# danielroe/ray-project-ray

Hardware: AMD Instinct MI355X
Metric: ray_train_gpt2_small_ddp_tokens_per_sec (higher is better)
Workload: dtype bf16

## Files before the change

### ray_amd/ops/_lib.py

```python

from __future__ import annotations

import ctypes
import os
import threading

_HERE = os.path.dirname(os.path.abspath(__file__))
LIB_PATH = os.path.join(os.path.dirname(_HERE), "_native", "libray_amd_hip.so")

_lib = None
_lock = threading.Lock()

c_void_p = ctypes.c_void_p
c_int = ctypes.c_int
c_long = ctypes.c_long
c_float = ctypes.c_float
c_double = ctypes.c_double
c_size_t = ctypes.c_size_t

_SIGS = {
    "ra_layernorm_fwd": [c_void_p] * 6 + [c_int, c_int, c_float, c_void_p],
    "ra_layernorm_bwd_parts": [c_int],
    "ra_layernorm_bwd": [c_void_p] * 11 + [c_int, c_int, c_int, c_void_p],
    "ra_residual_layernorm_fwd": [c_void_p] * 9 + [c_int, c_int, c_float, c_void_p],
# ... 34 lines not shown
    "ra_ppo_loss": [c_void_p] * 10 + [c_int, c_int] + [c_float] * 5 + [c_int, c_void_p],
    "ra_ppo_loss_packed": [c_void_p, c_void_p, c_void_p, c_int, c_int] + [c_void_p] * 4
                          + [c_int, c_int] + [c_float] * 5 + [c_void_p, c_int, c_float, c_void_p],
    "ra_scale_to_bf16": [c_void_p, c_long, c_void_p, c_void_p, c_void_p],
    "ra_ppo_heads_fwd": [c_void_p, c_int] + [c_void_p] * 5 + [c_int, c_int] + [c_void_p] * 3
                        + [c_int, c_int] + [c_float] * 5 + [c_void_p, c_float, c_void_p],
    "ra_ppo_heads_work": [c_int, c_int],
    "ra_ppo_heads_bwd": [c_void_p, c_int] + [c_void_p] * 10 + [c_int, c_int, c_int, c_void_p],
    "ra_c51_loss": [c_void_p] * 13 + [c_int, c_int, c_int, c_float, c_float, c_void_p],
    "ra_bias_relu_fwd": [c_void_p, c_void_p, c_void_p, c_long, c_int, c_void_p],
    "ra_relu_bwd_work": [c_int, c_int],
    "ra_relu_bwd_bias": [c_void_p] * 5 + [c_int, c_int, c_int, c_void_p],
    "ra_obsnorm_parts": [c_int],
    "ra_obsnorm_update": [c_void_p, c_int, c_int, c_double, c_void_p, c_void_p, c_void_p,
                          c_void_p],
    "ra_obsnorm_apply": [c_void_p] * 4 + [c_long, c_int, c_double, c_float, c_float, c_void_p],
    "ra_lt_num_cands": [c_int, c_int] + [c_long] * 6,
    "ra_lt_release_stream": [c_void_p],
    "ra_embed_bwd": [c_void_p] * 6 + [c_int, c_int, c_int, c_int, c_void_p],
    "ra_embed_bwd_work": [c_int, c_int, c_int],
    "ra_lt_num_streams": [],
    "ra_lt_set_choice": [c_int, c_int] + [c_long] * 6 + [c_int],
    "ra_lt_gemm": [c_int, c_int, c_long, c_long, c_long, c_void_p, c_long, c_void_p, c_long,
                   c_void_p, c_long, c_float, c_float, c_void_p],
    "ra_lt_tune": [c_int, c_int, c_long, c_long, c_long, c_void_p, c_long, c_void_p, c_long,
                   c_void_p, c_long, c_int, c_void_p, c_int, c_long, c_long, c_long, c_void_p],
    "ra_lt_gemm_batched": [c_int, c_int, c_long, c_long, c_long, c_void_p, c_long, c_long,
                           c_void_p, c_long, c_long, c_void_p, c_long, c_long, c_int, c_float,
                           c_float, c_void_p],
    "ra_lt_ep_num_cands": [c_int, c_int] + [c_long] * 6 + [c_int, c_long],
    "ra_lt_ep_set_choice": [c_int, c_int] + [c_long] * 6 + [c_int, c_long, c_int],
    "ra_lt_gemm_ep": [c_int, c_int, c_long, c_long, c_long, c_void_p, c_long, c_void_p, c_long,
                      c_void_p, c_long, c_int, c_void_p, c_void_p, c_long, c_int, c_void_p],
    "ra_lt_num_cands_batched": [c_int, c_int] + [c_long] * 6 + [c_int, c_long, c_long, c_long],
    "ra_lt_set_choice_batched": [c_int, c_int] + [c_long] * 6 + [c_int, c_long, c_long, c_long,
                                                                  c_int],
    "ra_lt_choice_name": [c_int, c_int] + [c_long] * 6 + [c_int, c_long, c_long, c_long,
                                                           ctypes.c_char_p, c_int],
    "ra_lt_allow_streamk": [c_int],
    "ra_lt_choice_is_streamk": [c_int, c_int] + [c_long] * 6 + [c_int, c_long, c_long, c_long],
    "ra_image_normalize": [c_void_p, c_void_p, c_int, c_int, c_int, c_int, c_void_p, c_void_p,
                           c_int, c_void_p],
    "ra_resize_bilinear": [c_void_p, c_void_p] + [c_int] * 6 + [c_void_p],
    "ra_cast_scale_u8": [c_void_p, c_void_p, c_long, c_float, c_void_p],
    "ra_gather_cast_u8": [c_void_p, c_void_p, c_void_p, c_long, c_long, c_float, c_void_p],
    "ra_conv_supported": [c_int] * 6,
    "ra_conv_fwd": [c_void_p, c_void_p, c_int, c_void_p, c_void_p, c_void_p] + [c_int] * 8
                   + [c_float, c_int, c_void_p],
    "ra_conv_wgrad_work": [c_int] * 8,
    "ra_conv_dgrad_supported": [c_int] * 5,
    "ra_conv_dgrad": [c_void_p] * 3 + [c_int] * 8 + [c_void_p],
    "ra_conv_wgrad": [c_void_p, c_void_p, c_int, c_void_p, c_void_p, c_long, c_void_p, c_int]
                     + [c_int] * 8 + [c_float, c_void_p],
    "ra_attn_fwd": [c_void_p, c_void_p, c_void_p, c_int, c_int, c_int, c_int, c_float,
                    c_void_p],
    "ra_attn_bwd": [c_void_p] * 6 + [c_int, c_int, c_int, c_int, c_float, c_void_p],
    "ra_attn_decode_splits": [c_int, c_int, c_int],
    "ra_attn_decode_work": [c_int, c_int, c_int, c_int],
    "ra_attn_decode": [c_void_p] * 6 + [c_int, c_int, c_int, c_float, c_int, c_void_p],
    "ra_kv_insert": [c_void_p] * 5 + [c_int] * 5 + [c_void_p],
    "ra_kv_copy": [c_void_p] * 7 + [c_int] * 7 + [c_void_p],
    "ra_attn_extend": [c_void_p] * 7 + [c_int] * 5 + [c_float, c_void_p],
    "ra_lora_add": [c_void_p] * 6 + [c_int] * 6 + [c_void_p],
    "ra_slot_advance": [c_void_p] * 6 + [c_int, c_int, c_long, c_void_p],
    "ra_sample_logits_max_v": [],
    "ra_sample_logits": [c_void_p, c_long] + [c_void_p] * 6 + [c_int, c_void_p, c_int, c_int,
# ... 66 lines not shown
```

### ray_amd/ops/csrc/gemm_lt.hip

```cpp
#include "common.h"

#include <hipblaslt/hipblaslt.h>
#include <hipblaslt/hipblaslt-ext.hpp>

#include <cstdlib>
#include <cstring>
#include <map>
#include <mutex>
#include <string>
#include <tuple>
#include <vector>

namespace {

typedef std::tuple<int, int, long, long, long, long, long, long, int, long, long, long> LtKey;

struct LtPlan {
  hipblasLtMatmulDesc_t desc = nullptr;
  hipblasLtMatrixLayout_t a = nullptr, b = nullptr, c = nullptr;
  std::vector<hipblasLtMatmulHeuristicResult_t> cands;
  std::vector<signed char> streamk;
  bool sk_only = false;
  int choice = 0;
};

hipblasLtHandle_t g_handle = nullptr;
const size_t kWs = 64ull << 20;
std::map<LtKey, LtPlan*> g_plans;
std::mutex g_mu;
std::map<hipStream_t, void*> g_ws_by_stream;
std::map<hipStream_t, hipblasLtHandle_t> g_handle_by_stream;
std::mutex g_ws_mu;

bool env_on(const char* name) {
  const char* e = getenv(name);
  return e && e[0] == '1';
}

hipblasLtHandle_t handle_for(hipStream_t st) {
  static const bool shared = env_on("RAY_AMD_LT_SHARED_HANDLE");
  if (shared) return g_handle;
  std::lock_guard<std::mutex> lk(g_ws_mu);
  auto it = g_handle_by_stream.find(st);
  if (it != g_handle_by_stream.end()) return it->second;
  hipblasLtHandle_t h = nullptr;
  if (hipblasLtCreate(&h) != HIPBLAS_STATUS_SUCCESS) return g_handle;
  g_handle_by_stream[st] = h;
  return h;
}

void* workspace(hipStream_t st) {
  std::lock_guard<std::mutex> lk(g_ws_mu);
// ... 180 lines not shown
RA_EXPORT void ra_lt_allow_streamk(int on) {
  std::lock_guard<std::mutex> g(g_mu);
  g_allow_sk = on != 0;
}

RA_EXPORT int ra_lt_release_stream(void* stream) {
  hipStream_t st = (hipStream_t)stream;
  std::lock_guard<std::mutex> lk(g_ws_mu);
  int freed = 0;
  auto w = g_ws_by_stream.find(st);
  auto h = g_handle_by_stream.find(st);
  if (w == g_ws_by_stream.end() && h == g_handle_by_stream.end()) return 0;
  hipStreamSynchronize(st);
  if (w != g_ws_by_stream.end()) {
    hipFree(w->second);
    g_ws_by_stream.erase(w);
    ++freed;
  }
  if (h != g_handle_by_stream.end()) {
    if (h->second != g_handle) hipblasLtDestroy(h->second);
    g_handle_by_stream.erase(h);
    ++freed;
  }
  return freed;
}

RA_EXPORT int ra_lt_num_streams() {
  std::lock_guard<std::mutex> lk(g_ws_mu);
  return (int)(g_ws_by_stream.size() > g_handle_by_stream.size() ? g_ws_by_stream.size()
                                                                   : g_handle_by_stream.size());
}

namespace {
typedef std::tuple<int, int, long, long, long, long, long, long, int, long> EpKey;
std::map<EpKey, LtPlan*> g_ep_plans;

LtPlan* get_ep_plan(int ta, int tb, long m, long n, long k, long lda, long ldb, long ldd, int ep,
                    long ldaux) {
  const EpKey key(ta, tb, m, n, k, lda, ldb, ldd, ep, ldaux);
  auto it = g_ep_plans.find(key);
  if (it != g_ep_plans.end()) return it->second;
  if (init_handle() != 0) return nullptr;
  LtPlan* p = new LtPlan();
  hipblasLtMatmulDescCreate(&p->desc, HIPBLAS_COMPUTE_32F, HIP_R_32F);
  hipblasOperation_t oa = ta ? HIPBLAS_OP_T : HIPBLAS_OP_N, ob = tb ? HIPBLAS_OP_T : HIPBLAS_OP_N;
  hipblasLtMatmulDescSetAttribute(p->desc, HIPBLASLT_MATMUL_DESC_TRANSA, &oa, sizeof(oa));
  hipblasLtMatmulDescSetAttribute(p->desc, HIPBLASLT_MATMUL_DESC_TRANSB, &ob, sizeof(ob));
  uint32_t e = (uint32_t)ep;
  hipblasLtMatmulDescSetAttribute(p->desc, HIPBLASLT_MATMUL_DESC_EPILOGUE, &e, sizeof(e));
  int32_t bt = ep == HIPBLASLT_EPILOGUE_DGELU_BGRAD ? HIP_R_32F : HIP_R_16BF;
  hipblasLtMatmulDescSetAttribute(p->desc, HIPBLASLT_MATMUL_DESC_BIAS_DATA_TYPE, &bt, sizeof(bt));
  int64_t la = ldaux;
  hipblasLtMatmulDescSetAttribute(p->desc, HIPBLASLT_MATMUL_DESC_EPILOGUE_AUX_LD, &la, sizeof(la));
  hipblasLtMatrixLayoutCreate(&p->a, HIP_R_16BF, ta ? k : m, ta ? m : k, lda);
  hipblasLtMatrixLayoutCreate(&p->b, HIP_R_16BF, tb ? n : k, tb ? k : n, ldb);
  hipblasLtMatrixLayoutCreate(&p->c, HIP_R_16BF, m, n, ldd);
  hipblasLtMatmulPreference_t pref;
  hipblasLtMatmulPreferenceCreate(&pref);
  uint64_t wsz = kWs;
  hipblasLtMatmulPreferenceSetAttribute(pref, HIPBLASLT_MATMUL_PREF_MAX_WORKSPACE_BYTES, &wsz,
                                        sizeof(wsz));
  std::vector<hipblasLtMatmulHeuristicResult_t> res(64);
  int got = 0;
  hipblasLtMatmulAlgoGetHeuristic(g_handle, p->desc, p->a, p->b, p->c, p->c, pref, 64,
                                  res.data(), &got);
  hipblasLtMatmulPreferenceDestroy(pref);
  for (int i = 0; i < got; ++i)
    if (res[i].state == HIPBLAS_STATUS_SUCCESS && res[i].workspaceSize <= kWs)
      p->cands.push_back(res[i]);
  g_ep_plans[key] = p;
  return p;
}
}

RA_EXPORT int ra_lt_ep_num_cands(int ta, int tb, long m, long n, long k, long lda, long ldb,
                                 long ldd, int ep, long ldaux) {
  std::lock_guard<std::mutex> g(g_mu);
  LtPlan* p = get_ep_plan(ta, tb, m, n, k, lda, ldb, ldd, ep, ldaux);
  return p ? (int)p->cands.size() : -1;
}

RA_EXPORT int ra_lt_ep_set_choice(int ta, int tb, long m, long n, long k, long lda, long ldb,
                                  long ldd, int ep, long ldaux, int choice) {
  std::lock_guard<std::mutex> g(g_mu);
  LtPlan* p = get_ep_plan(ta, tb, m, n, k, lda, ldb, ldd, ep, ldaux);
  if (!p || choice < 0 || choice >= (int)p->cands.size()) return -1;
  p->choice = choice;
  return 0;
}

RA_EXPORT int ra_lt_gemm_ep(int ta, int tb, long m, long n, long k, const void* A, long lda,
                            const void* B, long ldb, void* D, long ldd, int ep, void* bias,
                            void* aux, long ldaux, int choice, hipStream_t st) {
  LtPlan* p;
  {
    std::lock_guard<std::mutex> g(g_mu);
    p = get_ep_plan(ta, tb, m, n, k, lda, ldb, ldd, ep, ldaux);
    if (!p || p->cands.empty()) return -1;
    hipblasLtMatmulDescSetAttribute(p->desc, HIPBLASLT_MATMUL_DESC_BIAS_POINTER, &bias,
                                    sizeof(bias));
    hipblasLtMatmulDescSetAttribute(p->desc, HIPBLASLT_MATMUL_DESC_EPILOGUE_AUX_POINTER, &aux,
                                    sizeof(aux));
  }
  const int idx = choice >= 0 && choice < (int)p->cands.size() ? choice : p->choice;
  const float alpha = 1.f, beta = 0.f;
  const hipblasStatus_t s =
      hipblasLtMatmul(handle_for(st), p->desc, &alpha, A, p->a, B, p->b, &beta, D, p->c, D,
                      p->c, &p->cands[idx].algo, workspace(st), kWs, st);
  return s == HIPBLAS_STATUS_SUCCESS ? 0 : 1000 + (int)s;
}

RA_EXPORT int ra_lt_tune(int ta, int tb, long m, long n, long k, const void* A, long lda,
                         const void* B, long ldb, float* scratch, long ldc, int iters,
                         float* best_ms, int batch, long sa, long sb, long sc, hipStream_t st) {
  std::lock_guard<std::mutex> g(g_mu);
  LtPlan* p = get_plan(ta, tb, m, n, k, lda, ldb, ldc, batch, sa, sb, sc);
  if (!p || p->cands.empty()) return -1;
  hipEvent_t e0, e1;
  hipEventCreate(&e0);
  hipEventCreate(&e1);
  int best = -1;
  float bt = 1e30f;
  for (int i = 0; i < (int)p->cands.size(); ++i) {
    if (!usable(p, i)) continue;
    if (run(p, i, A, B, scratch, 1.f, 0.f, st) != 0) continue;
    hipEventRecord(e0, st);
    bool ok = true;
    for (int r = 0; r < iters && ok; ++r) ok = run(p, i, A, B, scratch, 1.f, 0.f, st) == 0;
    hipEventRecord(e1, st);
    hipEventSynchronize(e1);
    float ms = 0.f;
    hipEventElapsedTime(&ms, e0, e1);
    if (ok && ms / iters < bt) {
      bt = ms / iters;
      best = i;
    }
  }
  hipEventDestroy(e0);
  hipEventDestroy(e1);
  if (best >= 0) p->choice = best;
// ... 4 lines not shown
```

### ray_amd/ops/functional.py

```python

from __future__ import annotations

import os

import torch

from . import _lib
from . import reference as ref
from ._lib import check, ptr, stream_ptr


def _hip(t: torch.Tensor) -> bool:
    return t.is_cuda


def _grad_sink(p):
    if p is not None and getattr(p, "_ra_direct_grad", False):
        return getattr(p, "_ra_grad", None)
    return None


def _sink_f32(t) -> int:
    return 1 if t is not None and t.dtype == torch.float32 else 0

# ... 361 lines not shown
                getattr(w, "_ra_wt_key", None) == (_weights_epoch[0], w._version):
            return view, getattr(w, "_ra_wt_ev", None)
        side = _side_stream(w.device)
        side.wait_stream(torch.cuda.current_stream(w.device))
        with torch.cuda.stream(side):
            check(_lib.lib().ra_transpose_bf16(ptr(w), ptr(view), w.shape[0], w.shape[1],
                                               side.cuda_stream), "transpose_bf16")
            ev = torch.cuda.Event()
            ev.record(side)
        w._ra_wt_key = (_weights_epoch[0], w._version)
        w._ra_wt_ev = ev
        return view, ev
    cache = getattr(w, "_ra_wt", None)
    key = (_weights_epoch[0], w._version, w.data_ptr())
    stale = cache is None or cache[1] != key or torch.cuda.is_current_stream_capturing()
    if not stale:
        return cache[0], cache[2]
    wt = cache[0] if cache is not None else torch.empty(w.shape[1], w.shape[0], dtype=w.dtype,
                                                        device=w.device)
    side = _side_stream(w.device)
    side.wait_stream(torch.cuda.current_stream(w.device))
    with torch.cuda.stream(side):
        if w.dtype == torch.bfloat16 and w.dim() == 2 and w.is_contiguous():
            check(_lib.lib().ra_transpose_bf16(ptr(w), ptr(wt), w.shape[0], w.shape[1],
                                               side.cuda_stream), "transpose_bf16")
        else:
            wt.copy_(w.detach().t())
        ev = torch.cuda.Event()
        ev.record(side)
    w._ra_wt = (wt, key, ev)
    return wt, ev


class _Linear(torch.autograd.Function):
    @staticmethod
    def forward(ctx, x, w, b):
        ctx.save_for_backward(x, w)
        ctx.b = b
        ctx.wt = _transposed_weight(w) if _DGRAD_WT and w.is_cuda and x.dim() >= 2 else None
        return torch.nn.functional.linear(x, w, b)

    @staticmethod
    def backward(ctx, dy):
        x, w = ctx.saved_tensors
        K, N = x.shape[-1], w.shape[0]
        x2 = x.reshape(-1, K)
        dy2 = dy.reshape(-1, N)
        M = x2.shape[0]
        dx = None
        if ctx.needs_input_grad[0]:
            if ctx.wt is not None:
                wt, ev = ctx.wt
                if ev is not None:
                    torch.cuda.current_stream(dy2.device).wait_event(ev)
                dx = (dy2 @ wt.t()).view(x.shape)
            else:
                dx = (dy2 @ w).view(x.shape)
        dw = db = None
        bsink = None
        if ctx.b is not None and ctx.needs_input_grad[2] and ctx.needs_input_grad[1]:
            bsink = _grad_sink(ctx.b)
            ws_ = _grad_sink(w)
            if bsink is not None and (ws_ is None or ws_.dtype != bsink.dtype):
                bsink = None
        if ctx.needs_input_grad[1]:
            sink = _grad_sink(w)
            S = _splitk(M, N, K)
            if sink is not None and _WGRAD_STREAM and dy2.is_cuda:
                _issue_side_wgrad((dy2, x2, w, sink, S, M, N, K, ctx.b, bsink))
            elif sink is not None:
                _wgrad_to_sink(dy2, x2, w, sink, S, M, N, K, ctx.b, bsink)
            elif S > 1:
                part = _wgrad_partials(dy2, x2, S, M, N, K)
                dw = torch.empty_like(w)
                check(_lib.lib().ra_splitk_accum(ptr(part), S, N * K, ptr(dw), 2 * _sink_f32(dw),
                                                 stream_ptr()), "splitk_accum")
            else:
                dw = dy2.t() @ x2
        if ctx.b is not None and ctx.needs_input_grad[2] and bsink is None:
            db = _bias_grad(dy2, ctx.b)
        return dx, dw, db


def linear(x, w, b=None):
    if _hip(x) and x.dtype == torch.bfloat16 and w.dtype == torch.bfloat16 and \
            (w.shape[0] * w.shape[1]) % 4 == 0:
        return _Linear.apply(x, w, b)
    return torch.nn.functional.linear(x, w, b)


class _FlashAttnQKV(torch.autograd.Function):
    @staticmethod
    def forward(ctx, qkv, scale):
        B, T, _, H, D = qkv.shape
        qkv = qkv.contiguous()
        out = torch.empty((B, T, H, D), device=qkv.device, dtype=qkv.dtype)
        lse = torch.empty((B, H, T), device=qkv.device, dtype=torch.float32)
        check(_lib.lib().ra_attn_fwd(ptr(qkv), ptr(out), ptr(lse), B, T, H, D, scale,
                                     stream_ptr()), "attn_fwd")
        ctx.save_for_backward(qkv, out, lse)
        ctx.scale = scale
        return out

    @staticmethod
    def backward(ctx, dout):
        qkv, out, lse = ctx.saved_tensors
        B, T, _, H, D = qkv.shape
        dout = dout.contiguous()
        dqkv = torch.empty_like(qkv)
        delta = torch.empty((B, H, T), device=qkv.device, dtype=torch.float32)
        check(_lib.lib().ra_attn_bwd(ptr(qkv), ptr(out), ptr(dout), ptr(lse), ptr(delta),
                                     ptr(dqkv), B, T, H, D, ctx.scale, stream_ptr()),
              "attn_bwd")
        return dqkv, None
# ... 988 lines not shown
```

### ray_amd/ops/lt.py

```python

from __future__ import annotations

import ctypes
import os
import threading

import torch

from . import _lib
from ._lib import check, ptr, stream_ptr

_HERE = os.path.dirname(os.path.abspath(__file__))
DEFAULT_FILE = os.path.join(os.path.dirname(_HERE), "tuned", "lt_f32out.csv")

_lock = threading.Lock()
_choices: dict | None = None
_applied: set = set()
_tuning = os.environ.get("RAY_AMD_LT_TUNE", "0") == "1"
_file = os.environ.get("RAY_AMD_LT_FILE", DEFAULT_FILE)


def set_tuning(on: bool, path: str | None = None):
    global _tuning, _file
    _tuning = bool(on)
# ... 82 lines not shown

def gemm_f32(ta: int, tb: int, m: int, n: int, k: int, A, lda: int, B, ldb: int, C, ldc: int,
             alpha: float = 1.0, beta: float = 0.0, batch: int = 1, sa: int = 0, sb: int = 0,
             sc: int = 0):
    _select(ta, tb, m, n, k, ptr(A), lda, ptr(B), ldb, ldc, C.device, batch, sa, sb, sc)
    if batch == 1:
        rc = _lib.lib().ra_lt_gemm(ta, tb, m, n, k, ptr(A), lda, ptr(B), ldb, ptr(C), ldc,
                                   float(alpha), float(beta), stream_ptr())
    else:
        rc = _lib.lib().ra_lt_gemm_batched(ta, tb, m, n, k, ptr(A), lda, sa, ptr(B), ldb, sb,
                                           ptr(C), ldc, sc, batch, float(alpha), float(beta),
                                           stream_ptr())
    check(rc, "lt_gemm")


def wgrad_partials(dy2: torch.Tensor, x2: torch.Tensor, S: int) -> torch.Tensor:
    M, N = dy2.shape
    K = x2.shape[1]
    Ms = M // S
    part = torch.empty((S, N, K), dtype=torch.float32, device=dy2.device)
    gemm_f32(0, 1, K, N, Ms, x2, K, dy2, N, part, K, batch=S, sa=Ms * K, sb=Ms * N, sc=N * K)
    return part


def wgrad_accum(dy2: torch.Tensor, x2: torch.Tensor, out: torch.Tensor, beta: float = 1.0,
                alpha: float = 1.0):
    M, N = dy2.shape
    K = x2.shape[1]
    assert x2.shape[0] == M and out.shape == (N, K) and out.dtype == torch.float32
    assert dy2.stride(1) == 1 and x2.stride(1) == 1 and out.is_contiguous()
    gemm_f32(0, 1, K, N, M, x2, x2.stride(0), dy2, dy2.stride(0), out, K, alpha, beta)


def release_stream(stream) -> int:
    from ._lib import lib

    return int(lib().ra_lt_release_stream(stream.cuda_stream))
```

### ray_amd/ops/csrc/attn.hip

```cpp
#include "attn_mfma.h"

#include <type_traits>

#define HD 64
#define TILE_ELEMS (64 * 64)

__device__ __forceinline__ int xcd_block(int bid, int n) {
  return (n & 7) ? bid : (bid & 7) * (n >> 3) + (bid >> 3);
}

struct PairedBlock {
  int i, bh;
  bool two;
  __device__ __forceinline__ PairedBlock(int L, int nb) {
    const int np = (nb + 1) / 2;
    i = L % np;
    bh = L / np;
    two = nb - 1 - i != i;
  }
};

struct QD {
  TileRegs q, d;
  float rc;
};

__device__ __forceinline__ void tile_load(TileRegs& r, const bf16_t* g, long gstride) {
  const int c = threadIdx.x;
  r.v0 = *reinterpret_cast<const u32x4*>(g + (c >> 3) * gstride + (c & 7) * 8);
  r.v1 = *reinterpret_cast<const u32x4*>(g + ((c + 256) >> 3) * gstride + (c & 7) * 8);
}

struct TileAddr {
  int voff0, voff1;
  __device__ __forceinline__ TileAddr(long gstride) {
    const int c = threadIdx.x;
    voff0 = (int)(((c >> 3) * gstride + (c & 7) * 8) * 2);
    voff1 = (int)((((c + 256) >> 3) * gstride + (c & 7) * 8) * 2);
  }
};
__device__ __forceinline__ void tile_load_buf(TileRegs& r, __amdgpu_buffer_rsrc_t rs,
                                              const TileAddr& a, int soff) {
  r.v0 = __builtin_bit_cast(u32x4, __builtin_amdgcn_raw_buffer_load_b128(rs, a.voff0, soff, 0));
  r.v1 = __builtin_bit_cast(u32x4, __builtin_amdgcn_raw_buffer_load_b128(rs, a.voff1, soff, 0));
}


__device__ __forceinline__ int opaque_lane(int lane) {
  asm volatile("" : "+v"(lane));
  return lane;
}

__device__ __forceinline__ void store_rows_lds(bf16_t* img, const f32x16 (&acc)[2], float mul,
                                               bf16_t* g0, long gstride, int lane) {
  const int r = lane & 31, hh = lane >> 5;
#pragma unroll
  for (int dt = 0; dt < 2; ++dt)
// ... 88 lines not shown
  load_kv(A, 0);
  load_kv(B, 1);
  for (bool more = pb.two;; more = false) {
    store_kv(A, 0);
    kv_move(A, B);
    __syncthreads();
    for (int t = 0; t < ntiles; t += 2) {
      step(t, A, B);
      if (t + 1 < ntiles) step(t + 1, B, A);
    }
    if (more) {
      load_q(qf, pb.i, opaque_lane(lane));
      load_kv(A, 0);
      load_kv(B, 1);
    }
    static_assert(4 * 2048 <= 2 * TILE_ELEMS, "O staging must fit one tile buffer");
    const float inv = 1.f / l_run;
    store_rows_lds(lds + 2 * TILE_ELEMS + w * 2048, o, inv,
                   out + ((long)b * T + wave_qmin) * C + h * HD, C, opaque_lane(lane));
    if (hh == 0) lse[(long)bh * T + qrow] = m_run + log2f(l_run);
    if (!more) break;
    qb = pb.i;
    set_block();
  }
}

__global__ __launch_bounds__(256) __attribute__((amdgpu_waves_per_eu(2, 2))) void attn_bwd_dkdv_kernel(
    const bf16_t* __restrict__ qkv, const bf16_t* __restrict__ dout,
    const float* __restrict__ lse, const float* __restrict__ delta, bf16_t* __restrict__ dqkv,
    int T, int H, float sc_log2, float scale) {
  __shared__ __attribute__((aligned(16))) bf16_t lds[2 * 2 * TILE_ELEMS + 2 * 2 * 64 * 2];
  float* rowc = reinterpret_cast<float*>(lds + 4 * TILE_ELEMS);
  const int nkb = T / 128;
  const int L = xcd_block(blockIdx.x, gridDim.x);
  const int kb = L % nkb;
  const int bh = L / nkb;
  const int b = bh / H, h = bh % H;
  const int C = H * HD;
  const long tok = 3L * C;
  const bf16_t* base = qkv + (long)b * T * tok + h * HD;
  const bf16_t* dobase = dout + (long)b * T * C + h * HD;
  const int w = threadIdx.x >> 6, lane = threadIdx.x & 63, r = lane & 31, hh = lane >> 5;
  const LaneOffs lo(lane);
  const int kv0 = kb * 128;
  const int key = kv0 + 32 * w + r;
  bf16x8_t kf[4], vf[4];
#pragma unroll
  for (int kk = 0; kk < 4; ++kk) {
    kf[kk] = ld8(base + C + (long)key * tok + 16 * kk + 8 * hh);
    vf[kk] = ld8(base + 2 * C + (long)key * tok + 16 * kk + 8 * hh);
  }
  f32x16 dv[2] = {}, dk[2] = {};
  const int t0 = kv0 / 64;
  const int ntiles = T / 64;
  const int wave_kmin = kv0 + 32 * w;
  const float inv_c = -1.f / sc_log2;
  const float* lse_bh = lse + (long)bh * T;
  const float* del_bh = delta + (long)bh * T;
  QD A;
  const __amdgpu_buffer_rsrc_t rq = __builtin_amdgcn_make_buffer_rsrc(
      (void*)base, 0, (T - 1) * (int)tok * 2 + 3 * C * 2, 0x00020000);
  const __amdgpu_buffer_rsrc_t rd = __builtin_amdgcn_make_buffer_rsrc(
      (void*)dobase, 0, T * C * 2, 0x00020000);
  const TileAddr taq(tok), tad(C);
  const __amdgpu_buffer_rsrc_t rl =
      __builtin_amdgcn_make_buffer_rsrc((void*)lse_bh, 0, T * 4, 0x00020000);
  const __amdgpu_buffer_rsrc_t rdl =
      __builtin_amdgcn_make_buffer_rsrc((void*)del_bh, 0, T * 4, 0x00020000);
  auto load_qd = [&](QD& x, int t) __attribute__((always_inline)) {
    tile_load_buf(x.q, rq, taq, t * 64 * (int)tok * 2);
    tile_load_buf(x.d, rd, tad, t * 64 * C * 2);
    if (threadIdx.x < 128) {
      const float v = __builtin_bit_cast(
          float, __builtin_amdgcn_raw_buffer_load_b32(threadIdx.x < 64 ? rl : rdl,
                                                      (t * 64 + (threadIdx.x & 63)) * 4, 0, 0));
      x.rc = threadIdx.x < 64 ? v * inv_c : -v;
    }
  };
  auto store_qd = [&](const QD& x, int t) __attribute__((always_inline)) {
    const int buf = (t - t0) & 1;
    bf16_t* d = lds + buf * 2 * TILE_ELEMS;
    tile_store(x.q, d);
    tile_store(x.d, d + TILE_ELEMS);
    if (threadIdx.x < 128) rowc[buf * 128 + threadIdx.x] = x.rc;
  };
  auto body = [&](int t, auto diag_c) __attribute__((always_inline)) {
    constexpr bool diag = decltype(diag_c)::value;
    const int cur = (t - t0) & 1;
    const int q0 = t * 64;
    const bf16_t* Qs = lds + cur * 2 * TILE_ELEMS;
    const bf16_t* Ds = Qs + TILE_ELEMS;
    const float* nl = rowc + cur * 128;
    const float* nd = nl + 64;
    f32x16 s[2], dp[2];
#pragma unroll
    for (int qt = 0; qt < 2; ++qt) {
#pragma unroll
      for (int g = 0; g < 4; ++g) {
        const float4 a = *reinterpret_cast<const float4*>(nl + 32 * qt + 8 * g + 4 * hh);
        const float4 d = *reinterpret_cast<const float4*>(nd + 32 * qt + 8 * g + 4 * hh);
        s[qt][4 * g] = a.x; s[qt][4 * g + 1] = a.y; s[qt][4 * g + 2] = a.z;
        s[qt][4 * g + 3] = a.w;
        dp[qt][4 * g] = d.x; dp[qt][4 * g + 1] = d.y; dp[qt][4 * g + 2] = d.z;
        dp[qt][4 * g + 3] = d.w;
      }
#pragma unroll
      for (int kk = 0; kk < 4; ++kk) {
        s[qt] = mfma32(ld8(Qs + 2048 * qt + lo.row[kk]), kf[kk], s[qt]);
        dp[qt] = mfma32(ld8(Ds + 2048 * qt + lo.row[kk]), vf[kk], dp[qt]);
      }
    }
#pragma unroll
    for (int qt = 0; qt < 2; ++qt) {
#pragma unroll
      for (int i = 0; i < 16; ++i) {
        float p = fast_exp2(s[qt][i] * sc_log2);
        if (diag && key > q0 + 32 * qt + crow(i, hh)) p = 0.f;
        s[qt][i] = p;
        dp[qt][i] = p * dp[qt][i];
      }
#pragma unroll
      for (int ks = 0; ks < 2; ++ks) {
        const bf16x8_t pa = acc_frag(s[qt], ks);
        const bf16x8_t da = acc_frag(dp[qt], ks);
        const int kbq = 32 * qt + 16 * ks;
#pragma unroll
        for (int dt = 0; dt < 2; ++dt) {
          dv[dt] = mfma32(pa, tr_frag(Ds, lo, kbq, dt), dv[dt]);
          dk[dt] = mfma32(da, tr_frag(Qs, lo, kbq, dt), dk[dt]);
        }
      }
    }
  };
  auto compute = [&](int t) __attribute__((always_inline)) {
    const int q0 = t * 64;
    if (q0 + 63 >= wave_kmin) {
      if (q0 < wave_kmin + 31) body(t, std::true_type{});
      else body(t, std::false_type{});
    }
  };
  load_qd(A, t0);
  store_qd(A, t0);
  __syncthreads();
  for (int t = t0; t < ntiles; ++t) {
    if (t + 1 < ntiles) load_qd(A, t + 1);
    compute(t);
    if (t + 1 < ntiles) store_qd(A, t + 1);
    __syncthreads();
  }
#pragma unroll
  for (int dt = 0; dt < 2; ++dt)
#pragma unroll
    for (int i = 0; i < 16; ++i) {
      const int kr = kv0 + 32 * w + crow(i, hh);
      bf16_t* g = dqkv + ((long)b * T + kr) * tok + h * HD + 32 * dt + r;
      g[C] = f2bf(dk[dt][i] * scale);
      g[2 * C] = f2bf(dv[dt][i]);
    }
}

__global__ __launch_bounds__(256) void attn_bwd_dq_kernel(
    const bf16_t* __restrict__ qkv, const bf16_t* __restrict__ dout,
    const float* __restrict__ lse, float* __restrict__ delta, bf16_t* __restrict__ dqkv,
    int T, int H, float sc_log2, float scale, const bf16_t* __restrict__ out) {
  __shared__ __attribute__((aligned(16))) bf16_t lds[2 * 2 * TILE_ELEMS];
  const int nqb = T / 128;
  const PairedBlock pb(xcd_block(blockIdx.x, gridDim.x), nqb);
  const int bh = pb.bh;
  const int b = bh / H, h = bh % H;
  const int C = H * HD;
  const long tok = 3L * C;
  const bf16_t* base = qkv + (long)b * T * tok + h * HD;
  const int w = threadIdx.x >> 6, lane = threadIdx.x & 63, r = lane & 31, hh = lane >> 5;
  const LaneOffs lo(lane);
  struct RowIn {
    bf16x8_t q[4], d[4], o[4];
    float lse;
  };
  auto load_rows = [&](RowIn& x, int blk, int ln) __attribute__((always_inline)) {
    const int row = blk * 128 + 32 * w + (ln & 31), c0 = 8 * (ln >> 5);
#pragma unroll
    for (int kk = 0; kk < 4; ++kk) {
      x.q[kk] = ld8(base + (long)row * tok + 16 * kk + c0);
      x.d[kk] = ld8(dout + ((long)b * T + row) * C + h * HD + 16 * kk + c0);
      x.o[kk] = ld8(out + ((long)b * T + row) * C + h * HD + 16 * kk + c0);
    }
    x.lse = lse[(long)bh * T + row];
  };
  int q0, qrow, ntiles, wave_qmax;
  bf16x8_t qf[4], df[4];
  float nlq, ndel;
// ... 96 lines not shown
    RowIn x;
    if (more) {
      load_rows(x, pb.i, opaque_lane(lane));
      load_kv(A, 0);
      load_kv(B, 1);
    }
    store_rows_lds(lds + 2 * TILE_ELEMS + w * 2048, dq, scale,
                   dqkv + ((long)b * T + q0 + 32 * w) * tok + h * HD, tok, opaque_lane(lane));
    if (!more) break;
    set_block(pb.i, x);
  }
}

static inline bool attn_shape_ok(int T, int D) { return D == HD && T % 128 == 0 && T >= 128; }
static inline int attn_grid(int B, int T, int H) { return B * H * ((T / 128 + 1) / 2); }

RA_EXPORT int ra_attn_fwd(const void* qkv, void* out, float* lse, int B, int T, int H, int D,
                          float scale, hipStream_t st) {
  if (!attn_shape_ok(T, D)) return hipErrorInvalidValue;
  const float sc_log2 = scale * 1.4426950408889634f;
  hipLaunchKernelGGL(attn_fwd_kernel, dim3(attn_grid(B, T, H)), dim3(256), 0, st,
                     (const bf16_t*)qkv, (bf16_t*)out, lse, T, H, sc_log2);
  return hipGetLastError();
}

RA_EXPORT int ra_attn_bwd(const void* qkv, const void* out, const void* dout, const float* lse,
                          float* delta, void* dqkv, int B, int T, int H, int D, float scale,
                          hipStream_t st) {
  if (!attn_shape_ok(T, D)) return hipErrorInvalidValue;
  const float sc_log2 = scale * 1.4426950408889634f;
  hipLaunchKernelGGL(attn_bwd_dq_kernel, dim3(attn_grid(B, T, H)), dim3(256), 0, st,
                     (const bf16_t*)qkv, (const bf16_t*)dout, lse, delta, (bf16_t*)dqkv, T, H,
                     sc_log2, scale, (const bf16_t*)out);
  hipLaunchKernelGGL(attn_bwd_dkdv_kernel, dim3(B * H * (T / 128)), dim3(256), 0, st,
                     (const bf16_t*)qkv, (const bf16_t*)dout, lse, delta, (bf16_t*)dqkv, T, H,
                     sc_log2, scale);
  return hipGetLastError();
}
```

### ray_amd/ops/csrc/wgrad.hip

```cpp
#include "common.h"

namespace {

typedef __bf16 bf16x8w_t __attribute__((ext_vector_type(8)));
typedef __bf16 bf16x4w_t __attribute__((ext_vector_type(4)));
typedef __bf16 bf16x2w_t __attribute__((ext_vector_type(2)));
typedef short s16x4w_t __attribute__((ext_vector_type(4)));
typedef float f32x4w_t __attribute__((ext_vector_type(4)));
typedef __attribute__((address_space(3))) void lds_void_w;
typedef __attribute__((address_space(1))) void glb_void_w;

constexpr int kT = 64;
constexpr int kTile = 256;
constexpr int kImg = kT * kTile;
constexpr int kStage = 2 * kImg;
constexpr int kThreads = 512;

__device__ __forceinline__ int fsw(int r) { return (r & 3) | ((r >> 1) & 4); }

__device__ __forceinline__ bf16x4w_t tr4(const bf16_t* p) {
  typedef __attribute__((address_space(3))) s16x4w_t lds_s16x4;
  s16x4w_t v = __builtin_amdgcn_ds_read_tr16_b64_v4i16((lds_s16x4*)const_cast<bf16_t*>(p));
  return __builtin_bit_cast(bf16x4w_t, v);
}

__device__ __forceinline__ int xcd_remap_w(int b, int G) {
  const int q = G / 8, rr = G % 8, x = b % 8;
  return (x < rr ? x * (q + 1) : rr * (q + 1) + (x - rr) * q) + b / 8;
}

__device__ __forceinline__ void glds16_w(const bf16_t* gsrc, bf16_t* ldst) {
  const unsigned la = __builtin_amdgcn_readfirstlane(
      (unsigned)(unsigned long)(__attribute__((address_space(3))) void*)ldst);
  unsigned saved;
  asm volatile(
      "s_mov_b32 %0, m0\n\t"
      "s_mov_b32 m0, %2\n\t"
      "s_nop 0\n\t"
      "global_load_lds_dwordx4 %1, off\n\t"
      "s_mov_b32 m0, %0"
      : "=&s"(saved)
      : "v"(gsrc), "s"(la)
      : "memory");
}

template <int N>
__device__ __forceinline__ void wait_vm_w() {
  asm volatile("s_waitcnt vmcnt(%0)" ::"n"(N) : "memory");
}

struct WgradArgs {
  const bf16_t* dy;
  const bf16_t* x;
  long ldy, ldx;
  void* out;
  float* bias_out;
  int N, K, nks;
  int S, tk_cnt, ntiles;
  int flags;
};

__device__ __forceinline__ void stage_t(bf16_t* img, const bf16_t* __restrict__ g, long ld,
                                        int col0, int cols, long t0, int w, int lane) {
  const int rsub = lane >> 5, cp = lane & 31;
#pragma unroll
  for (int j = 0; j < 4; ++j) {
    const int r = 8 * w + 2 * j + rsub;
    const int c = cp ^ (2 * fsw(r));
    int col = col0 + 8 * c;
    col = col < cols ? col : cols - 8;
    const bf16_t* src = g + (t0 + r) * ld + col;
    glds16_w(src, img + (8 * w + 2 * j) * kTile);
  }
}

struct TileJob {
  const bf16_t* dy;
  const bf16_t* x;
  long ldy, ldx;
  int N, K, n0, k0, s_beg, total;
  bool do_bias;
};
// ... 276 lines not shown
```

Measured before the change: 1.066 million.

## Add hipBLASLt GEMM with bias and residual-add epilogue for linear layers

Adds a hipBLASLt matmul path that computes out = W·y + bias + skip in one call, using beta=1 with a separate C input layout and a bias epilogue. The autograd function and the linear_residual helper let projection layers fold the residual add into the GEMM. The aim is to remove a separate bias-plus-residual elementwise kernel and its memory traffic. The backward pass reuses the shared linear backward and passes dy through to the skip input. It adds candidate tuning and plan caching keyed on ldc.

Result: slower. 879,500 (-17.5%).

```diff
diff --git a/ray_amd/ops/_lib.py b/ray_amd/ops/_lib.py
--- a/ray_amd/ops/_lib.py
+++ b/ray_amd/ops/_lib.py
@@ -90,6 +90,10 @@
     "ra_lt_ep_set_choice": [c_int, c_int] + [c_long] * 6 + [c_int, c_long, c_int],
     "ra_lt_gemm_ep": [c_int, c_int, c_long, c_long, c_long, c_void_p, c_long, c_void_p, c_long,
                       c_void_p, c_long, c_int, c_void_p, c_void_p, c_long, c_int, c_void_p],
+    "ra_lt_res_num_cands": [c_int, c_int] + [c_long] * 7,
+    "ra_lt_res_set_choice": [c_int, c_int] + [c_long] * 7 + [c_int],
+    "ra_lt_gemm_res": [c_int, c_int, c_long, c_long, c_long, c_void_p, c_long, c_void_p, c_long,
+                       c_void_p, c_long, c_void_p, c_long, c_void_p, c_int, c_void_p],
     "ra_lt_num_cands_batched": [c_int, c_int] + [c_long] * 6 + [c_int, c_long, c_long, c_long],
     "ra_lt_set_choice_batched": [c_int, c_int] + [c_long] * 6 + [c_int, c_long, c_long, c_long,
                                                                   c_int],
diff --git a/ray_amd/ops/csrc/gemm_lt.hip b/ray_amd/ops/csrc/gemm_lt.hip
--- a/ray_amd/ops/csrc/gemm_lt.hip
+++ b/ray_amd/ops/csrc/gemm_lt.hip
@@ -18,6 +18,7 @@
 struct LtPlan {
   hipblasLtMatmulDesc_t desc = nullptr;
   hipblasLtMatrixLayout_t a = nullptr, b = nullptr, c = nullptr;
+  hipblasLtMatrixLayout_t cin = nullptr;
   std::vector<hipblasLtMatmulHeuristicResult_t> cands;
   std::vector<signed char> streamk;
   bool sk_only = false;
@@ -264,12 +265,12 @@
 }
 
 namespace {
-typedef std::tuple<int, int, long, long, long, long, long, long, int, long> EpKey;
+typedef std::tuple<int, int, long, long, long, long, long, long, int, long, long> EpKey;
 std::map<EpKey, LtPlan*> g_ep_plans;
 
 LtPlan* get_ep_plan(int ta, int tb, long m, long n, long k, long lda, long ldb, long ldd, int ep,
-                    long ldaux) {
-  const EpKey key(ta, tb, m, n, k, lda, ldb, ldd, ep, ldaux);
+                    long ldaux, long ldc = 0) {
+  const EpKey key(ta, tb, m, n, k, lda, ldb, ldd, ep, ldaux, ldc);
   auto it = g_ep_plans.find(key);
   if (it != g_ep_plans.end()) return it->second;
   if (init_handle() != 0) return nullptr;
@@ -283,10 +284,13 @@
   int32_t bt = ep == HIPBLASLT_EPILOGUE_DGELU_BGRAD ? HIP_R_32F : HIP_R_16BF;
   hipblasLtMatmulDescSetAttribute(p->desc, HIPBLASLT_MATMUL_DESC_BIAS_DATA_TYPE, &bt, sizeof(bt));
   int64_t la = ldaux;
-  hipblasLtMatmulDescSetAttribute(p->desc, HIPBLASLT_MATMUL_DESC_EPILOGUE_AUX_LD, &la, sizeof(la));
+  if (ldaux > 0)
+    hipblasLtMatmulDescSetAttribute(p->desc, HIPBLASLT_MATMUL_DESC_EPILOGUE_AUX_LD, &la,
+                                    sizeof(la));
   hipblasLtMatrixLayoutCreate(&p->a, HIP_R_16BF, ta ? k : m, ta ? m : k, lda);
   hipblasLtMatrixLayoutCreate(&p->b, HIP_R_16BF, tb ? n : k, tb ? k : n, ldb);
   hipblasLtMatrixLayoutCreate(&p->c, HIP_R_16BF, m, n, ldd);
+  if (ldc > 0) hipblasLtMatrixLayoutCreate(&p->cin, HIP_R_16BF, m, n, ldc);
   hipblasLtMatmulPreference_t pref;
   hipblasLtMatmulPreferenceCreate(&pref);
   uint64_t wsz = kWs;
@@ -294,8 +298,8 @@
                                         sizeof(wsz));
   std::vector<hipblasLtMatmulHeuristicResult_t> res(64);
   int got = 0;
-  hipblasLtMatmulAlgoGetHeuristic(g_handle, p->desc, p->a, p->b, p->c, p->c, pref, 64,
-                                  res.data(), &got);
+  hipblasLtMatmulAlgoGetHeuristic(g_handle, p->desc, p->a, p->b, p->cin ? p->cin : p->c, p->c,
+                                  pref, 64, res.data(), &got);
   hipblasLtMatmulPreferenceDestroy(pref);
   for (int i = 0; i < got; ++i)
     if (res[i].state == HIPBLAS_STATUS_SUCCESS && res[i].workspaceSize <= kWs)
@@ -338,6 +342,41 @@
   const float alpha = 1.f, beta = 0.f;
   const hipblasStatus_t s =
       hipblasLtMatmul(handle_for(st), p->desc, &alpha, A, p->a, B, p->b, &beta, D, p->c, D,
+                      p->c, &p->cands[idx].algo, workspace(st), kWs, st);
+  return s == HIPBLAS_STATUS_SUCCESS ? 0 : 1000 + (int)s;
+}
+
+static const int kResEp = HIPBLASLT_EPILOGUE_BIAS;
+
+RA_EXPORT int ra_lt_res_num_cands(int ta, int tb, long m, long n, long k, long lda, long ldb,
+                                  long ldc, long ldd) {
+  std::lock_guard<std::mutex> g(g_mu);
+  LtPlan* p = ldc > 0 ? get_ep_plan(ta, tb, m, n, k, lda, ldb, ldd, kResEp, 0, ldc) : nullptr;
+  return p ? (int)p->cands.size() : -1;
+}
+
+RA_EXPORT int ra_lt_res_set_choice(int ta, int tb, long m, long n, long k, long lda, long ldb,
+                                   long ldc, long ldd, int choice) {
+  std::lock_guard<std::mutex> g(g_mu);
+  LtPlan* p = ldc > 0 ? get_ep_plan(ta, tb, m, n, k, lda, ldb, ldd, kResEp, 0, ldc) : nullptr;
+  if (!p || choice < 0 || choice >= (int)p->cands.size()) return -1;
+  p->choice = choice;
+  return 0;
+}
+
+RA_EXPORT int ra_lt_gemm_res(int ta, int tb, long m, long n, long k, const void* A, long lda,
+                             const void* B, long ldb, const void* C, long ldc, void* D, long ldd,
+                             const void* bias, int choice, hipStream_t st) {
+  if (ldc <= 0 || !A || !B || !C || !D || !bias || D == C) return -1;
+  std::lock_guard<std::mutex> g(g_mu);
+  LtPlan* p = get_ep_plan(ta, tb, m, n, k, lda, ldb, ldd, kResEp, 0, ldc);
+  if (!p || p->cands.empty()) return -1;
+  hipblasLtMatmulDescSetAttribute(p->desc, HIPBLASLT_MATMUL_DESC_BIAS_POINTER, &bias,
+                                  sizeof(bias));
+  const int idx = choice >= 0 && choice < (int)p->cands.size() ? choice : p->choice;
+  const float alpha = 1.f, beta = 1.f;
+  const hipblasStatus_t s =
+      hipblasLtMatmul(handle_for(st), p->desc, &alpha, A, p->a, B, p->b, &beta, C, p->cin, D,
                       p->c, &p->cands[idx].algo, workspace(st), kWs, st);
   return s == HIPBLAS_STATUS_SUCCESS ? 0 : 1000 + (int)s;
 }
diff --git a/ray_amd/ops/functional.py b/ray_amd/ops/functional.py
--- a/ray_amd/ops/functional.py
+++ b/ray_amd/ops/functional.py
@@ -417,6 +417,47 @@
     return wt, ev
 
 
+def _linear_backward(ctx, dy):
+    x, w = ctx.saved_tensors
+    K, N = x.shape[-1], w.shape[0]
+    x2 = x.reshape(-1, K)
+    dy2 = dy.reshape(-1, N)
+    M = x2.shape[0]
+    dx = None
+    if ctx.needs_input_grad[0]:
+        if ctx.wt is not None:
+            wt, ev = ctx.wt
+            if ev is not None:
+                torch.cuda.current_stream(dy2.device).wait_event(ev)
+            dx = (dy2 @ wt.t()).view(x.shape)
+        else:
+            dx = (dy2 @ w).view(x.shape)
+    dw = db = None
+    bsink = None
+    if ctx.b is not None and ctx.needs_input_grad[2] and ctx.needs_input_grad[1]:
+        bsink = _grad_sink(ctx.b)
+        ws_ = _grad_sink(w)
+        if bsink is not None and (ws_ is None or ws_.dtype != bsink.dtype):
+            bsink = None
+    if ctx.needs_input_grad[1]:
+        sink = _grad_sink(w)
+        S = _splitk(M, N, K)
+        if sink is not None and _WGRAD_STREAM and dy2.is_cuda:
+            _issue_side_wgrad((dy2, x2, w, sink, S, M, N, K, ctx.b, bsink))
+        elif sink is not None:
+            _wgrad_to_sink(dy2, x2, w, sink, S, M, N, K, ctx.b, bsink)
+        elif S > 1:
+            part = _wgrad_partials(dy2, x2, S, M, N, K)
+            dw = torch.empty_like(w)
+            check(_lib.lib().ra_splitk_accum(ptr(part), S, N * K, ptr(dw), 2 * _sink_f32(dw),
+                                             stream_ptr()), "splitk_accum")
+        else:
+            dw = dy2.t() @ x2
+    if ctx.b is not None and ctx.needs_input_grad[2] and bsink is None:
+        db = _bias_grad(dy2, ctx.b)
+    return dx, dw, db
+
+
 class _Linear(torch.autograd.Function):
     @staticmethod
     def forward(ctx, x, w, b):
@@ -427,44 +468,45 @@
 
     @staticmethod
     def backward(ctx, dy):
-        x, w = ctx.saved_tensors
-        K, N = x.shape[-1], w.shape[0]
-        x2 = x.reshape(-1, K)
-        dy2 = dy.reshape(-1, N)
-        M = x2.shape[0]
-        dx = None
-        if ctx.needs_input_grad[0]:
-            if ctx.wt is not None:
-                wt, ev = ctx.wt
-                if ev is not None:
-                    torch.cuda.current_stream(dy2.device).wait_event(ev)
-                dx = (dy2 @ wt.t()).view(x.shape)
-            else:
-                dx = (dy2 @ w).view(x.shape)
-        dw = db = None
-        bsink = None
-        if ctx.b is not None and ctx.needs_input_grad[2] and ctx.needs_input_grad[1]:
-            bsink = _grad_sink(ctx.b)
-            ws_ = _grad_sink(w)
-            if bsink is not None and (ws_ is None or ws_.dtype != bsink.dtype):
-                bsink = None
-        if ctx.needs_input_grad[1]:
-            sink = _grad_sink(w)
-            S = _splitk(M, N, K)
-            if sink is not None and _WGRAD_STREAM and dy2.is_cuda:
-                _issue_side_wgrad((dy2, x2, w, sink, S, M, N, K, ctx.b, bsink))
-            elif sink is not None:
-                _wgrad_to_sink(dy2, x2, w, sink, S, M, N, K, ctx.b, bsink)
-            elif S > 1:
-                part = _wgrad_partials(dy2, x2, S, M, N, K)
-                dw = torch.empty_like(w)
-                check(_lib.lib().ra_splitk_accum(ptr(part), S, N * K, ptr(dw), 2 * _sink_f32(dw),
-                                                 stream_ptr()), "splitk_accum")
-            else:
-                dw = dy2.t() @ x2
-        if ctx.b is not None and ctx.needs_input_grad[2] and bsink is None:
-            db = _bias_grad(dy2, ctx.b)
-        return dx, dw, db
+        return _linear_backward(ctx, dy)
+
+
+class _LinearResidual(torch.autograd.Function):
+
+    @staticmethod
+    def forward(ctx, y, w, b, skip):
+        from . import lt
+
+        ctx.save_for_backward(y, w)
+        ctx.b = b
+        ctx.wt = _transposed_weight(w) if _DGRAD_WT else None
+        out = lt.gemm_bias_residual(y.reshape(-1, y.shape[-1]), w, b,
+                                    skip.reshape(-1, w.shape[0]))
+        return out.view(skip.shape)
+
+    @staticmethod
+    def backward(ctx, dy):
+        return _linear_backward(ctx, dy) + (dy,)
+
+
+def linear_residual_ok(y, w, b, skip) -> bool:
+    if not (_hip(y) and b is not None and w.dim() == 2 and y.dim() >= 2
+            and y.dtype == w.dtype == b.dtype == skip.dtype == torch.bfloat16
+            and skip.is_cuda and y.shape[-1] == w.shape[1] and skip.shape[-1] == w.shape[0]
+            and skip.shape[:-1] == y.shape[:-1]
+            and y.is_contiguous() and w.is_contiguous() and skip.is_contiguous()
+            and b.is_contiguous() and w.shape[0] % 8 == 0 and w.shape[1] % 8 == 0):
+        return False
+    from . import lt
+
+    return lt.residual_ready(y.numel() // y.shape[-1], w.shape[0], w.shape[1])
+
+
+def linear_residual(y, w, b, skip):
+    if linear_residual_ok(y, w, b, skip):
+        return _LinearResidual.apply(y, w, b, skip)
+    h = linear(y, w)
+    return bias_residual(h, b, skip) if b is not None else h + skip
 
 
 def linear(x, w, b=None):
diff --git a/ray_amd/ops/lt.py b/ray_amd/ops/lt.py
--- a/ray_amd/ops/lt.py
+++ b/ray_amd/ops/lt.py
@@ -138,6 +138,75 @@
     gemm_f32(0, 1, K, N, M, x2, x2.stride(0), dy2, dy2.stride(0), out, K, alpha, beta)
 
 
+def _res_shape(M: int, N: int, K: int):
+    return (1, 0, N, M, K, K, K, N, N)
+
+
+def _res_key(shape) -> str:
+    return "lt_res_" + "_".join(map(str, shape[2:]))
+
+
+def residual_num_cands(M: int, N: int, K: int) -> int:
+    return int(_lib.lib().ra_lt_res_num_cands(*_res_shape(M, N, K)))
+
+
+def residual_ready(M: int, N: int, K: int) -> bool:
+    if residual_num_cands(M, N, K) <= 0:
+        return False
+    return _res_key(_res_shape(M, N, K)) in _applied or \
+        not torch.cuda.is_current_stream_capturing()
+
+
+def _select_res(shape, key, a2, w, bias, skip2, out):
+    if key in _applied:
+        return
+    with _lock:
+        if key in _applied:
+            return
+        L = _lib.lib()
+        nc = L.ra_lt_res_num_cands(*shape)
+        if nc <= 0:
+            raise RuntimeError(f"hipBLASLt has no solution for {key}")
+        ch = _load()
+        if key in ch and ch[key][0] < nc and L.ra_lt_res_set_choice(*shape, ch[key][0]) == 0:
+            pass
+        elif _tuning:
+            ta, tb, m, n, k, lda, ldb, ldc, ldd = shape
+            args = (ta, tb, m, n, k, ptr(w), lda, ptr(a2), ldb, ptr(skip2), ldc, ptr(out), ldd,
+                    ptr(bias))
+            best, best_ms = -1, float("inf")
+            e0, e1 = torch.cuda.Event(enable_timing=True), torch.cuda.Event(enable_timing=True)
+            for i in range(nc):
+                if L.ra_lt_gemm_res(*args, i, stream_ptr()) != 0:
+                    continue
+                e0.record()
+                ok = all(L.ra_lt_gemm_res(*args, i, stream_ptr()) == 0 for _ in range(5))
+                e1.record()
+                e1.synchronize()
+                if ok and e0.elapsed_time(e1) / 5 < best_ms:
+                    best, best_ms = i, e0.elapsed_time(e1) / 5
+            if best >= 0 and L.ra_lt_res_set_choice(*shape, best) == 0:
+                ch[key] = (best, best_ms)
+        _applied.add(key)
+
+
+def gemm_bias_residual(a2: torch.Tensor, w: torch.Tensor, bias: torch.Tensor,
+                       skip2: torch.Tensor) -> torch.Tensor:
+    M, K = a2.shape
+    N = w.shape[0]
+    assert w.shape == (N, K) and bias.shape == (N,) and skip2.shape == (M, N)
+    assert a2.is_contiguous() and w.is_contiguous() and skip2.is_contiguous() and \
+        bias.is_contiguous()
+    assert a2.dtype == w.dtype == bias.dtype == skip2.dtype == torch.bfloat16
+    out = torch.empty_like(skip2)
+    shape = _res_shape(M, N, K)
+    _select_res(shape, _res_key(shape), a2, w, bias, skip2, out)
+    ta, tb, m, n, k, lda, ldb, ldc, ldd = shape
+    check(_lib.lib().ra_lt_gemm_res(ta, tb, m, n, k, ptr(w), lda, ptr(a2), ldb, ptr(skip2), ldc,
+                                    ptr(out), ldd, ptr(bias), -1, stream_ptr()), "lt_gemm_res")
+    return out
+
+
 def release_stream(stream) -> int:
     from ._lib import lib
 
```

## Pair causal key blocks and stream Q/dO tiles via LDS DMA in dK/dV kernel

Applied to the files above, without the earlier changes.

Reworks the attention backward dK/dV kernel so each workgroup handles a pair of key blocks (i and nkb-1-i), which balances the causal triangle's uneven work and halves the grid. Q and dO tiles now go from global memory straight into LDS through global_load_lds DMA instead of passing through registers, and the next block's K/V fragments and first tile are prefetched while the current block's results are written out. The shared DMA helpers move into a common header. The risks are correctness of the swizzled DMA addressing and of the partial vmcnt wait, plus lower parallelism from the smaller grid.

After: 1.070 million tokens/s before, 1.077 million tokens/s after, median of 6. Within noise of the previous version (+0.7%).

```diff
diff --git a/ray_amd/ops/csrc/attn.hip b/ray_amd/ops/csrc/attn.hip
--- a/ray_amd/ops/csrc/attn.hip
+++ b/ray_amd/ops/csrc/attn.hip
@@ -1,4 +1,5 @@
 #include "attn_mfma.h"
+#include "lds_dma.h"
 
 #include <type_traits>
 
@@ -18,11 +19,6 @@
     bh = L / np;
     two = nb - 1 - i != i;
   }
-};
-
-struct QD {
-  TileRegs q, d;
-  float rc;
 };
 
 __device__ __forceinline__ void tile_load(TileRegs& r, const bf16_t* g, long gstride) {
@@ -177,57 +173,61 @@
   __shared__ __attribute__((aligned(16))) bf16_t lds[2 * 2 * TILE_ELEMS + 2 * 2 * 64 * 2];
   float* rowc = reinterpret_cast<float*>(lds + 4 * TILE_ELEMS);
   const int nkb = T / 128;
-  const int L = xcd_block(blockIdx.x, gridDim.x);
-  const int kb = L % nkb;
-  const int bh = L / nkb;
+  const PairedBlock pb(xcd_block(blockIdx.x, gridDim.x), nkb);
+  const int bh = pb.bh;
   const int b = bh / H, h = bh % H;
   const int C = H * HD;
   const long tok = 3L * C;
   const bf16_t* base = qkv + (long)b * T * tok + h * HD;
   const bf16_t* dobase = dout + (long)b * T * C + h * HD;
-  const int w = threadIdx.x >> 6, lane = threadIdx.x & 63, r = lane & 31, hh = lane >> 5;
+  const int w = threadIdx.x >> 6;
+  const int wu = __builtin_amdgcn_readfirstlane(w);
+  const int lane = threadIdx.x & 63, r = lane & 31, hh = lane >> 5;
   const LaneOffs lo(lane);
-  const int kv0 = kb * 128;
-  const int key = kv0 + 32 * w + r;
+  const int ntiles = T / 64;
+  const float inv_c = -1.f / sc_log2;
+  int kv0, key, t0, wave_kmin;
   bf16x8_t kf[4], vf[4];
-#pragma unroll
-  for (int kk = 0; kk < 4; ++kk) {
-    kf[kk] = ld8(base + C + (long)key * tok + 16 * kk + 8 * hh);
-    vf[kk] = ld8(base + 2 * C + (long)key * tok + 16 * kk + 8 * hh);
-  }
-  f32x16 dv[2] = {}, dk[2] = {};
-  const int t0 = kv0 / 64;
-  const int ntiles = T / 64;
-  const int wave_kmin = kv0 + 32 * w;
-  const float inv_c = -1.f / sc_log2;
-  const float* lse_bh = lse + (long)bh * T;
-  const float* del_bh = delta + (long)bh * T;
-  QD A;
-  const __amdgpu_buffer_rsrc_t rq = __builtin_amdgcn_make_buffer_rsrc(
-      (void*)base, 0, (T - 1) * (int)tok * 2 + 3 * C * 2, 0x00020000);
-  const __amdgpu_buffer_rsrc_t rd = __builtin_amdgcn_make_buffer_rsrc(
-      (void*)dobase, 0, T * C * 2, 0x00020000);
-  const TileAddr taq(tok), tad(C);
-  const __amdgpu_buffer_rsrc_t rl =
-      __builtin_amdgcn_make_buffer_rsrc((void*)lse_bh, 0, T * 4, 0x00020000);
-  const __amdgpu_buffer_rsrc_t rdl =
-      __builtin_amdgcn_make_buffer_rsrc((void*)del_bh, 0, T * 4, 0x00020000);
-  auto load_qd = [&](QD& x, int t) __attribute__((always_inline)) {
-    tile_load_buf(x.q, rq, taq, t * 64 * (int)tok * 2);
-    tile_load_buf(x.d, rd, tad, t * 64 * C * 2);
-    if (threadIdx.x < 128) {
-      const float v = __builtin_bit_cast(
-          float, __builtin_amdgcn_raw_buffer_load_b32(threadIdx.x < 64 ? rl : rdl,
-                                                      (t * 64 + (threadIdx.x & 63)) * 4, 0, 0));
-      x.rc = threadIdx.x < 64 ? v * inv_c : -v;
-    }
-  };
-  auto store_qd = [&](const QD& x, int t) __attribute__((always_inline)) {
-    const int buf = (t - t0) & 1;
-    bf16_t* d = lds + buf * 2 * TILE_ELEMS;
-    tile_store(x.q, d);
-    tile_store(x.d, d + TILE_ELEMS);
-    if (threadIdx.x < 128) rowc[buf * 128 + threadIdx.x] = x.rc;
+  f32x16 dv[2], dk[2];
+  auto set_block = [&](int kb) __attribute__((always_inline)) {
+    kv0 = kb * 128;
+    key = kv0 + 32 * w + r;
+    t0 = kv0 / 64;
+    wave_kmin = kv0 + 32 * w;
+    dv[0] = dv[1] = dk[0] = dk[1] = f32x16{};
+  };
+  auto load_kvf = [&](int kb, int ln) __attribute__((always_inline)) {
+    const bf16_t* g = base + (long)(kb * 128 + 32 * w + (ln & 31)) * tok + 8 * (ln >> 5);
+#pragma unroll
+    for (int kk = 0; kk < 4; ++kk) {
+      kf[kk] = ld8(g + C + 16 * kk);
+      vf[kk] = ld8(g + 2 * C + 16 * kk);
+    }
+  };
+  const int srow = 16 * w + (lane >> 3);
+  const unsigned sq0 = (unsigned)(srow * (int)tok * 2) + (((lane & 7) ^ swz(srow)) << 4);
+  const unsigned sq1 = (unsigned)((srow + 8) * (int)tok * 2) + (((lane & 7) ^ swz(srow + 8)) << 4);
+  const unsigned sd0 = (unsigned)(srow * C * 2) + (((lane & 7) ^ swz(srow)) << 4);
+  const unsigned sd1 = (unsigned)((srow + 8) * C * 2) + (((lane & 7) ^ swz(srow + 8)) << 4);
+  const __amdgpu_buffer_rsrc_t rrc = __builtin_amdgcn_make_buffer_rsrc(
+      (void*)((wu == 0 ? lse : delta) + (long)bh * T), 0, T * 4, 0x00020000);
+  const unsigned lds0 = lds_addr(lds) + 16 * wu * 64 * 2;
+  auto dma_qd = [&](int t, int first) __attribute__((always_inline)) {
+    const unsigned d = lds0 + ((t - first) & 1) * 2 * TILE_ELEMS * 2;
+    const bf16_t* gq = base + (long)t * 64 * tok;
+    const bf16_t* gd = dobase + (long)t * 64 * C;
+    glds16_s(gq, sq0, d);
+    glds16_s(gq, sq1, d + 8 * 64 * 2);
+    glds16_s(gd, sd0, d + TILE_ELEMS * 2);
+    glds16_s(gd, sd1, d + TILE_ELEMS * 2 + 8 * 64 * 2);
+  };
+  auto load_rc = [&](float& rc, int t) __attribute__((always_inline)) {
+    if (wu < 2)
+      rc = __builtin_bit_cast(
+          float, __builtin_amdgcn_raw_buffer_load_b32(rrc, (t * 64 + lane) * 4, 0, 0));
+  };
+  auto store_rc = [&](float rc, int t, int first) __attribute__((always_inline)) {
+    if (wu < 2) rowc[((t - first) & 1) * 128 + 64 * wu + lane] = wu == 0 ? rc * inv_c : -rc;
   };
   auto body = [&](int t, auto diag_c) __attribute__((always_inline)) {
     constexpr bool diag = decltype(diag_c)::value;
@@ -284,24 +284,59 @@
       else body(t, std::false_type{});
     }
   };
-  load_qd(A, t0);
-  store_qd(A, t0);
+  auto kvf_landed = [&]() __attribute__((always_inline)) {
+#pragma unroll
+    for (int kk = 0; kk < 4; ++kk)
+      asm volatile("" ::"v"(__builtin_bit_cast(u32x4, kf[kk])),
+                   "v"(__builtin_bit_cast(u32x4, vf[kk])));
+  };
+  float rc;
+  set_block(pb.i);
+  load_kvf(pb.i, lane);
+  dma_qd(t0, t0);
+  load_rc(rc, t0);
+  store_rc(rc, t0, t0);
+  wait_vm_w<0>();
+  kvf_landed();
   __syncthreads();
-  for (int t = t0; t < ntiles; ++t) {
-    if (t + 1 < ntiles) load_qd(A, t + 1);
-    compute(t);
-    if (t + 1 < ntiles) store_qd(A, t + 1);
+  for (bool more = pb.two;; more = false) {
+    for (int t = t0; t < ntiles; ++t) {
+      const bool nx = t + 1 < ntiles;
+      if (nx) {
+        dma_qd(t + 1, t0);
+        load_rc(rc, t + 1);
+      }
+      compute(t);
+      if (nx) store_rc(rc, t + 1, t0);
+      wait_vm_w<0>();
+      __syncthreads();
+    }
+    const int so = kv0;
+    if (more) {
+      const int nb = nkb - 1 - pb.i;
+      load_kvf(nb, opaque_lane(lane));
+      dma_qd(2 * nb, 2 * nb);
+      load_rc(rc, 2 * nb);
+    }
+    {
+      const int ln = opaque_lane(lane);
+      bf16_t* g0 = dqkv + ((long)b * T + so + 32 * w + 4 * (ln >> 5)) * tok + h * HD + (ln & 31);
+#pragma unroll
+      for (int dt = 0; dt < 2; ++dt)
+#pragma unroll
+        for (int i = 0; i < 16; ++i) {
+          bf16_t* g = g0 + ((i & 3) + 8 * (i >> 2)) * tok + 32 * dt;
+          g[C] = f2bf(dk[dt][i] * scale);
+          g[2 * C] = f2bf(dv[dt][i]);
+        }
+    }
+    if (!more) break;
+    set_block(nkb - 1 - pb.i);
+    store_rc(rc, t0, t0);
+    wait_vm_w<62>();
+    kvf_landed();
     __syncthreads();
   }
-#pragma unroll
-  for (int dt = 0; dt < 2; ++dt)
-#pragma unroll
-    for (int i = 0; i < 16; ++i) {
-      const int kr = kv0 + 32 * w + crow(i, hh);
-      bf16_t* g = dqkv + ((long)b * T + kr) * tok + h * HD + 32 * dt + r;
-      g[C] = f2bf(dk[dt][i] * scale);
-      g[2 * C] = f2bf(dv[dt][i]);
-    }
 }
 
 __global__ __launch_bounds__(256) void attn_bwd_dq_kernel(
@@ -464,7 +499,7 @@
   hipLaunchKernelGGL(attn_bwd_dq_kernel, dim3(attn_grid(B, T, H)), dim3(256), 0, st,
                      (const bf16_t*)qkv, (const bf16_t*)dout, lse, delta, (bf16_t*)dqkv, T, H,
                      sc_log2, scale, (const bf16_t*)out);
-  hipLaunchKernelGGL(attn_bwd_dkdv_kernel, dim3(B * H * (T / 128)), dim3(256), 0, st,
+  hipLaunchKernelGGL(attn_bwd_dkdv_kernel, dim3(attn_grid(B, T, H)), dim3(256), 0, st,
                      (const bf16_t*)qkv, (const bf16_t*)dout, lse, delta, (bf16_t*)dqkv, T, H,
                      sc_log2, scale);
   return hipGetLastError();
diff --git a/ray_amd/ops/csrc/lds_dma.h b/ray_amd/ops/csrc/lds_dma.h
--- /dev/null
+++ b/ray_amd/ops/csrc/lds_dma.h
@@ -0,0 +1,39 @@
+#pragma once
+#include "common.h"
+
+__device__ __forceinline__ void glds16_w(const bf16_t* gsrc, bf16_t* ldst) {
+  const unsigned la = __builtin_amdgcn_readfirstlane(
+      (unsigned)(unsigned long)(__attribute__((address_space(3))) void*)ldst);
+  unsigned saved;
+  asm volatile(
+      "s_mov_b32 %0, m0\n\t"
+      "s_mov_b32 m0, %2\n\t"
+      "s_nop 0\n\t"
+      "global_load_lds_dwordx4 %1, off\n\t"
+      "s_mov_b32 m0, %0"
+      : "=&s"(saved)
+      : "v"(gsrc), "s"(la)
+      : "memory");
+}
+
+__device__ __forceinline__ unsigned lds_addr(const void* p) {
+  return (unsigned)(unsigned long)(__attribute__((address_space(3))) const void*)p;
+}
+
+__device__ __forceinline__ void glds16_s(const bf16_t* sbase, unsigned voff, unsigned ldst) {
+  unsigned saved;
+  asm volatile(
+      "s_mov_b32 %0, m0\n\t"
+      "s_mov_b32 m0, %3\n\t"
+      "s_nop 0\n\t"
+      "global_load_lds_dwordx4 %1, %2\n\t"
+      "s_mov_b32 m0, %0"
+      : "=&s"(saved)
+      : "v"(voff), "s"(sbase), "s"(ldst)
+      : "memory");
+}
+
+template <int N>
+__device__ __forceinline__ void wait_vm_w() {
+  asm volatile("s_waitcnt vmcnt(%0)" ::"n"(N) : "memory");
+}
diff --git a/ray_amd/ops/csrc/wgrad.hip b/ray_amd/ops/csrc/wgrad.hip
--- a/ray_amd/ops/csrc/wgrad.hip
+++ b/ray_amd/ops/csrc/wgrad.hip
@@ -1,4 +1,5 @@
 #include "common.h"
+#include "lds_dma.h"
 
 namespace {
 
@@ -29,25 +30,6 @@
   return (x < rr ? x * (q + 1) : rr * (q + 1) + (x - rr) * q) + b / 8;
 }
 
-__device__ __forceinline__ void glds16_w(const bf16_t* gsrc, bf16_t* ldst) {
-  const unsigned la = __builtin_amdgcn_readfirstlane(
-      (unsigned)(unsigned long)(__attribute__((address_space(3))) void*)ldst);
-  unsigned saved;
-  asm volatile(
-      "s_mov_b32 %0, m0\n\t"
-      "s_mov_b32 m0, %2\n\t"
-      "s_nop 0\n\t"
-      "global_load_lds_dwordx4 %1, off\n\t"
-      "s_mov_b32 m0, %0"
-      : "=&s"(saved)
-      : "v"(gsrc), "s"(la)
-      : "memory");
-}
-
-template <int N>
-__device__ __forceinline__ void wait_vm_w() {
-  asm volatile("s_waitcnt vmcnt(%0)" ::"n"(N) : "memory");
-}
 
 struct WgradArgs {
   const bf16_t* dy;
```
